# google/speedy

Hardware: AMD Instinct MI355X
Metric: Msamples/s processed (16 kHz mono, 3.5x nonlinear) (higher is better)
Workload: dtype int16 samples; f64 DFT, f32 features, int32 AMDF/OLA

## Files before the change

### speedy_amd/csrc/spx_analysis.hip

```cpp
#include <stdlib.h>

#include "spx_internal.h"
#include "spx_walk_common.h"

#ifndef SPX_TF
#define SPX_TF 16
#endif

#ifdef SPX_STAMPS
__device__ unsigned long long g_spx_astamps[16];
#define ASTAMP_DECL unsigned long long as_last = __builtin_readcyclecounter(), as_acc[10] = {0,0,0,0,0,0,0,0,0,0};
#define ASTAMP(i) do { const unsigned long long t_ = __builtin_readcyclecounter(); as_acc[i] += t_ - as_last; as_last = t_; } while (0)
#define ASTAMP_FLUSH if (threadIdx.x == 0 && blockIdx.x == 7) for (int i_ = 0; i_ < 10; i_++) g_spx_astamps[i_] += as_acc[i_];
extern "C" void spx_debug_astamps(unsigned long long* out, int reset) {
  (void)hipMemcpyFromSymbol(out, HIP_SYMBOL(g_spx_astamps), sizeof(unsigned long long) * 16);
  if (reset) { unsigned long long z[16] = {0}; (void)hipMemcpyToSymbol(HIP_SYMBOL(g_spx_astamps), z, sizeof(z)); }
}
#else
#define ASTAMP_DECL
#define ASTAMP(i)
#define ASTAMP_FLUSH
#endif

#ifndef SPX_TF_SMALL
#define SPX_TF_SMALL 8
#endif
#define SPX_TF_TINY 4
int spx_analysis_tile_frames() { return SPX_TF; }
int spx_analysis_small_tile_frames() { return SPX_TF_SMALL; }
int spx_analysis_tiny_tile_frames() { return SPX_TF_TINY; }

#define SPX_CB 24
static __host__ __device__ constexpr int spx_mag_stride(int W) { return (W + 4) & ~3; }
static __host__ __device__ constexpr int spx_cb(int tf) { return tf <= 8 ? 2 * SPX_CB : SPX_CB; }
#ifdef SPX_LOG_V1
#define SPX_LOG_LDS_BYTES 0
#else
#define SPX_LOG_LDS_BYTES 2048
#endif
static __host__ __device__ inline size_t terms_bytes(int W, int tf, bool ct) {
  const size_t b = ct ? (size_t)2 * tf * (spx_cb(tf) + 1) * sizeof(double)
                      : (size_t)tf * (W + 1) * sizeof(double);
  return (b + 15) & ~(size_t)15;
}
static __host__ __device__ inline size_t work_bytes(int W, int tf, bool ct = false, int dft_waves = 4) {
  if (dft_waves < 1 || dft_waves > 4) dft_waves = 4;
  const size_t a = ct ? (size_t)4 * 2 * W * sizeof(double)
                      : (size_t)dft_waves * 2 * 2 * W * sizeof(double);
  const size_t b = terms_bytes(W, tf, ct) + SPX_LOG_LDS_BYTES;
  return (a > b ? a : b);
}
static inline int plan_ct_window(const SpxPlanDev& P) {
  auto is = [](const int* r, int n, std::initializer_list<int> want) {
    if (n != (int)want.size()) return false;
    int k = 0;
    for (int w : want) if (r[k++] != w) return false;
    return true;
  };
  if (!P.rader && P.W == 240 && is(P.radix, P.nstages, {4, 4, 3, 5})) return 240;
  if (!P.rader && P.W == 330 && is(P.radix, P.nstages, {2, 3, 5, 11})) return 330;
  if (P.tile_frames == SPX_TF_SMALL && P.dft_waves == 4) {
    if (!P.rader && P.W == 720 && is(P.radix, P.nstages, {4, 4, 3, 3, 5})) return 720;
    if (P.rader && P.W == 661 && is(P.radixM, P.nstagesM, {4, 3, 5, 11})) return 661;
  }
  if (!P.rader && P.dft_waves == 4) {
    if (P.W == 120 && is(P.radix, P.nstages, {4, 2, 3, 5}) && (P.tile_frames == SPX_TF || P.tile_frames == SPX_TF_SMALL)) return 120;
    if (P.W == 180 && is(P.radix, P.nstages, {4, 3, 3, 5}) && P.tile_frames == SPX_TF) return 180;
    if (P.W == 360 && is(P.radix, P.nstages, {4, 2, 3, 3, 5}) && P.tile_frames == SPX_TF) return 360;
    if (P.W == 480 && is(P.radix, P.nstages, {4, 4, 2, 3, 5}) && P.tile_frames == SPX_TF) return 480;
  }
  return 0;
}
int spx_analysis_prefers_small_tile(const SpxPlanDev& P) {
  SpxPlanDev Q = P;
  Q.tile_frames = SPX_TF_SMALL;
  Q.dft_waves = 4;
  const int w = plan_ct_window(Q);
  return w == 720 || w == 661;
}
static __host__ __device__ inline size_t stage_samples(const SpxPlanDev& P, int tf) {
  return (size_t)(tf + 1) * P.B + (P.W - P.B) + 8;
}
static size_t analysis_lds_bytes(const SpxPlanDev& P, bool ct) {
  const int tf = P.tile_frames > 0 ? P.tile_frames : SPX_TF;
  size_t mags = (size_t)(tf + 1) * spx_mag_stride(P.W) * sizeof(float);
  size_t small = (size_t)3 * (tf + 1) * sizeof(float);
  size_t stage = (stage_samples(P, tf) * sizeof(short) + 15) & ~(size_t)15;
  return work_bytes(P.W, tf, ct, P.dft_waves) + ((mags + 15) & ~(size_t)15) + ((small + 15) & ~(size_t)15) + stage;
}
size_t spx_analysis_lds_bytes(const SpxPlanDev& P) { return analysis_lds_bytes(P, plan_ct_window(P) != 0); }
int spx_analysis_ct_window(const SpxPlanDev& P) { return plan_ct_window(P); }

__device__ __forceinline__ void wave_sync() {
  __builtin_amdgcn_fence(__ATOMIC_RELEASE, "wavefront");
  __builtin_amdgcn_wave_barrier();
  __builtin_amdgcn_fence(__ATOMIC_ACQUIRE, "wavefront");
}

#include "spx_log.h"

__device__ __forceinline__ float spx_untangle_mag(double ar, double ai, double b_r, double b_i, double2 w) {
  const double dr = ar - b_r, di = ai - b_i;
#ifdef SPX_DFT_V1
  const double er = 0.5 * (ar + b_r), ei = 0.5 * (ai + b_i);
  const double o_r = 0.5 * di, o_i = -0.5 * dr;
  const double xr = er + (w.x * o_r - w.y * o_i);
  const double xi = ei + (w.x * o_i + w.y * o_r);
  return spx_sqrt64_to_f32(xr * xr + xi * xi);
#else
  const double xr2 = __builtin_fma(w.x, di, __builtin_fma(w.y, dr, ar + b_r));
  const double xi2 = __builtin_fma(w.y, di, __builtin_fma(-w.x, dr, ai + b_i));
  return spx_sqrt64_to_f32(0.25 * __builtin_fma(xr2, xr2, xi2 * xi2));
#endif
}

#define C5_1 0.30901699437494742
#define C5_2 (-0.80901699437494742)
#define S5_1 0.95105651629515357
#define S5_2 0.58778525229247313
#define S3_1 0.86602540378443865

struct cplx {
  double r, i;
};

#ifdef SPX_DFT_V1
#define SPX_FMA_OR(a, b, c, unfused) (unfused)
#else
#define SPX_FMA_OR(a, b, c, unfused) __builtin_fma((a), (b), (c))
#endif
__host__ __device__ __forceinline__ cplx spx_cmul(cplx b, double wx, double wy) {
  return {SPX_FMA_OR(b.r, wx, -(b.i * wy), b.r * wx - b.i * wy), SPX_FMA_OR(b.r, wy, b.i * wx, b.r * wy + b.i * wx)};
}
__host__ __device__ __forceinline__ double spx_bf3h(double a0, double t1) { return SPX_FMA_OR(-0.5, t1, a0, a0 - 0.5 * t1); }
__host__ __device__ __forceinline__ double spx_bf5m(double a0, double c1, double t1, double c2, double t2) {
  return SPX_FMA_OR(c2, t2, __builtin_fma(c1, t1, a0), (a0 + c1 * t1) + c2 * t2);
}
__host__ __device__ __forceinline__ double spx_bf5n(double s1, double t3, double s2, double t4) { return SPX_FMA_OR(s1, t3, s2 * t4, s1 * t3 + s2 * t4); }
__host__ __device__ __forceinline__ double spx_bf5d(double s2, double t3, double s1, double t4) { return SPX_FMA_OR(s2, t3, -(s1 * t4), s2 * t3 - s1 * t4); }
__host__ __device__ __forceinline__ double spx_acc(double p, double w, double u) { return SPX_FMA_OR(w, u, p, p + w * u); }

__host__ __device__ __forceinline__ cplx ld(const double* buf, int idx) {
  const double2 v = *reinterpret_cast<const double2*>(buf + 2 * idx);
  return {v.x, v.y};
}
__host__ __device__ __forceinline__ void st_tw(double* buf, int idx, cplx b, const double* tw, int t) {
  const double2 w = *reinterpret_cast<const double2*>(tw + 2 * t);
  const cplx v = spx_cmul(b, w.x, w.y);
  *reinterpret_cast<double2*>(buf + 2 * idx) = make_double2(v.r, v.i);
}

__host__ __device__ void dft_stage(const int W, const double* tw, int r, int s, int cur, const double* x, double* y,
                                   int lane, const int nl) {
  const int m = cur / r;
  const int span = W / r;
  const unsigned inv_s = ((1u << 20) + (unsigned)s - 1u) / (unsigned)s;
  if (r == 4) {
    for (int b = lane; b < span; b += nl) {
      const int p = (int)(((unsigned)b * inv_s) >> 20), q = b - p * s;
      cplx a0 = ld(x, b), a1 = ld(x, b + span), a2 = ld(x, b + 2 * span), a3 = ld(x, b + 3 * span);
      cplx t0 = {a0.r + a2.r, a0.i + a2.i}, t1 = {a0.r - a2.r, a0.i - a2.i};
      cplx t2 = {a1.r + a3.r, a1.i + a3.i}, t3 = {a1.r - a3.r, a1.i - a3.i};
      cplx b0 = {t0.r + t2.r, t0.i + t2.i}, b2 = {t0.r - t2.r, t0.i - t2.i};
      cplx b1 = {t1.r + t3.i, t1.i - t3.r}, b3 = {t1.r - t3.i, t1.i + t3.r};
      const int o = q + s * 4 * p;
      const int tp = s * p;
      st_tw(y, o, b0, tw, 0);
      st_tw(y, o + s, b1, tw, tp);
      st_tw(y, o + 2 * s, b2, tw, 2 * tp);
      st_tw(y, o + 3 * s, b3, tw, 3 * tp);
    }
  } else if (r == 2) {
    for (int b = lane; b < span; b += nl) {
      const int p = (int)(((unsigned)b * inv_s) >> 20), q = b - p * s;
      cplx a0 = ld(x, b), a1 = ld(x, b + span);
      cplx b0 = {a0.r + a1.r, a0.i + a1.i}, b1 = {a0.r - a1.r, a0.i - a1.i};
      const int o = q + s * 2 * p;
      st_tw(y, o, b0, tw, 0);
      st_tw(y, o + s, b1, tw, s * p);
    }
  } else if (r == 3) {
    for (int b = lane; b < span; b += nl) {
      const int p = (int)(((unsigned)b * inv_s) >> 20), q = b - p * s;
      cplx a0 = ld(x, b), a1 = ld(x, b + span), a2 = ld(x, b + 2 * span);
      cplx t1 = {a1.r + a2.r, a1.i + a2.i};
      cplx t2 = {spx_bf3h(a0.r, t1.r), spx_bf3h(a0.i, t1.i)};
      cplx t3 = {S3_1 * (a1.r - a2.r), S3_1 * (a1.i - a2.i)};
      cplx b0 = {a0.r + t1.r, a0.i + t1.i};
      cplx b1 = {t2.r + t3.i, t2.i - t3.r}, b2 = {t2.r - t3.i, t2.i + t3.r};
      const int o = q + s * 3 * p;
      const int tp = s * p;
      st_tw(y, o, b0, tw, 0);
      st_tw(y, o + s, b1, tw, tp);
      st_tw(y, o + 2 * s, b2, tw, 2 * tp);
    }
  } else if (r == 5) {
    for (int b = lane; b < span; b += nl) {
      const int p = (int)(((unsigned)b * inv_s) >> 20), q = b - p * s;
      cplx a0 = ld(x, b), a1 = ld(x, b + span), a2 = ld(x, b + 2 * span), a3 = ld(x, b + 3 * span),
           a4 = ld(x, b + 4 * span);
      cplx t1 = {a1.r + a4.r, a1.i + a4.i}, t2 = {a2.r + a3.r, a2.i + a3.i};
      cplx t3 = {a1.r - a4.r, a1.i - a4.i}, t4 = {a2.r - a3.r, a2.i - a3.i};
      cplx b0 = {(a0.r + t1.r) + t2.r, (a0.i + t1.i) + t2.i};
      cplx m1 = {spx_bf5m(a0.r, C5_1, t1.r, C5_2, t2.r), spx_bf5m(a0.i, C5_1, t1.i, C5_2, t2.i)};
      cplx m2 = {spx_bf5m(a0.r, C5_2, t1.r, C5_1, t2.r), spx_bf5m(a0.i, C5_2, t1.i, C5_1, t2.i)};
      cplx n1 = {spx_bf5n(S5_1, t3.r, S5_2, t4.r), spx_bf5n(S5_1, t3.i, S5_2, t4.i)};
      cplx n2 = {spx_bf5d(S5_2, t3.r, S5_1, t4.r), spx_bf5d(S5_2, t3.i, S5_1, t4.i)};
      cplx b1 = {m1.r + n1.i, m1.i - n1.r}, b4 = {m1.r - n1.i, m1.i + n1.r};
      cplx b2 = {m2.r + n2.i, m2.i - n2.r}, b3 = {m2.r - n2.i, m2.i + n2.r};
      const int o = q + s * 5 * p;
      const int tp = s * p;
      st_tw(y, o, b0, tw, 0);
      st_tw(y, o + s, b1, tw, tp);
      st_tw(y, o + 2 * s, b2, tw, 2 * tp);
      st_tw(y, o + 3 * s, b3, tw, 3 * tp);
      st_tw(y, o + 4 * s, b4, tw, 4 * tp);
    }
  } else {
    const int step = W / r;
    const int h = (r - 1) >> 1;
    for (int item = lane; item < span * h; item += nl) {
      const int b = item / h, j = item - b * h + 1;
      const int p = (int)(((unsigned)b * inv_s) >> 20), q = b - p * s;
      const cplx a0 = ld(x, b);
      cplx P = a0, Q = {0.0, 0.0}, B0 = a0;
      int t = 0;
      for (int i = 1; i <= h; i++) {
        t += j;
        t -= (t >= r) ? r : 0;
        const cplx ai = ld(x, b + i * span), ar = ld(x, b + (r - i) * span);
        const cplx u = {ai.r + ar.r, ai.i + ar.i}, v = {ai.r - ar.r, ai.i - ar.i};
        const double2 w = *reinterpret_cast<const double2*>(tw + 2 * (t * step));
        B0.r = B0.r + u.r; B0.i = B0.i + u.i;
        P.r = spx_acc(P.r, w.x, u.r); P.i = spx_acc(P.i, w.x, u.i);
        if (i == 1) { Q.r = w.y * v.r; Q.i = w.y * v.i; }
        else { Q.r = spx_acc(Q.r, w.y, v.r); Q.i = spx_acc(Q.i, w.y, v.i); }
      }
      const cplx bj = {P.r - Q.i, P.i + Q.r}, brj = {P.r + Q.i, P.i - Q.r};
      const int o = q + s * r * p;
      st_tw(y, o + s * j, bj, tw, s * p * j);
      st_tw(y, o + s * (r - j), brj, tw, s * p * (r - j));
      if (j == 1) st_tw(y, o, B0, tw, 0);
    }
  }
  (void)m;
}

void spx_host_dft(int n, const int* radix, int nstages, const double* tw, const double* in, double* out) {
  double* a = new double[4 * (size_t)n];
  double* x = a;
  double* y = a + 2 * (size_t)n;
  for (int i = 0; i < 2 * n; i++) x[i] = in[i];
  int s = 1, cur = n;
  for (int st = 0; st < nstages; st++) {
    dft_stage(n, tw, radix[st], s, cur, x, y, 0, 1);
    double* t = x; x = y; y = t;
    s *= radix[st];
    cur /= radix[st];
  }
  for (int i = 0; i < 2 * n; i++) out[i] = x[i];
  delete[] a;
}

__device__ __forceinline__ int mono_sample(const int16_t* __restrict__ in, int64_t a, int C) {
  if (C == 1) return in[a];
  int sum = 0;
  const int16_t* p = in + a * C;
  for (int c = 0; c < C; c++) sum += p[c];
  return sum / C;
}

__device__ __forceinline__ cplx cmul_tw(cplx b, double2 w) { return spx_cmul(b, w.x, w.y); }
__device__ __forceinline__ void st(double* buf, int idx, cplx v) {
  *reinterpret_cast<double2*>(buf + 2 * idx) = make_double2(v.r, v.i);
}

template <int R>
// ... 72 lines not shown
    constexpr int SPAN = NPTS / R;
    const int b = (lane + 64 * u < SPAN) ? lane + 64 * u : 0;
    return ld(buf, b + i * SPAN);
  }
};

template <int W, int ST, int S>
__device__ __forceinline__ void ct_stages_from(double* buf, const double2* __restrict__ twp, const int lane) {
  if constexpr (ST < ct_plan<W>::n) {
    constexpr int R = ct_plan<W>::r[ST];
    ct_stage<W, R, S>(buf, twp, lane, ct_from_buf<W, R>{buf, lane});
    ct_stages_from<W, ST + 1, S * R>(buf, twp, lane);
  }
}

template <int NPTS, int R>
__device__ __forceinline__ void ct_stage_prime_last(double* buf, const int lane, const double (&wc)[R - 1], const double (&ws)[R - 1]) {
  constexpr int SPAN = NPTS / R, H = (R - 1) / 2;
  static_assert(SPAN <= 64, "one pass");
  if (lane < SPAN) {
    cplx a[R];
#pragma unroll
    for (int i = 0; i < R; i++) a[i] = ld(buf, lane + SPAN * i);
    cplx uu[H], vv[H];
    cplx B0 = a[0];
#pragma unroll
    for (int i = 1; i <= H; i++) {
      uu[i - 1] = {a[i].r + a[R - i].r, a[i].i + a[R - i].i};
      vv[i - 1] = {a[i].r - a[R - i].r, a[i].i - a[R - i].i};
      B0.r = B0.r + uu[i - 1].r; B0.i = B0.i + uu[i - 1].i;
    }
    st(buf, lane, B0);
#pragma unroll
    for (int jj = 1; jj <= H; jj++) {
      cplx Pj = a[0], Qj = {0.0, 0.0};
#pragma unroll
      for (int i = 1; i <= H; i++) {
        const double wx = wc[(i * jj) % R - 1], wy = ws[(i * jj) % R - 1];
        Pj.r = spx_acc(Pj.r, wx, uu[i - 1].r); Pj.i = spx_acc(Pj.i, wx, uu[i - 1].i);
        if (i == 1) { Qj.r = wy * vv[0].r; Qj.i = wy * vv[0].i; }
        else { Qj.r = spx_acc(Qj.r, wy, vv[i - 1].r); Qj.i = spx_acc(Qj.i, wy, vv[i - 1].i); }
      }
      st(buf, lane + SPAN * jj, cplx{Pj.r - Qj.i, Pj.i + Qj.r});
      st(buf, lane + SPAN * (R - jj), cplx{Pj.r + Qj.i, Pj.i - Qj.r});
    }
  }
  wave_sync();
}

template <class T>
__device__ __forceinline__ const T* per_frame(const T* p) {
  asm volatile("" : "+s"(p));
  return p;
}
__device__ __forceinline__ double uniform_f64(double v) {
  return __longlong_as_double(((long long)__builtin_amdgcn_readfirstlane((int)(__double_as_longlong(v) >> 32)) << 32) |
                              (unsigned)__builtin_amdgcn_readfirstlane((int)__double_as_longlong(v)));
}

#ifdef SPX_PREEMPH_V1
#define SPX_WIN_SCALE 1.0f
__device__ __forceinline__ float spx_preemph_win_f32(double md, double mpd, float w) {
  const float x = (float)(md / 32768.0), xp = (float)(mpd / 32768.0);
  const float y = (float)(1.0 * (double)x - 0.97 * (double)xp);
  return y * w;
}
#else
#define SPX_WIN_SCALE 0x1p-15f
__device__ __forceinline__ float spx_preemph_win_f32(double md, double mpd, float w15) {
  const float yy = (float)(md - 0.97 * mpd);
  return yy * w15;
}
#endif
__device__ __forceinline__ double spx_preemph_win(double md, double mpd, float w) { return (double)spx_preemph_win_f32(md, mpd, w); }
__device__ __forceinline__ cplx packed_point(const short* fr, int n, int j, int prev0, float w0, float w1) {
  const int i0 = 2 * n;
  const int m0 = fr[i0], m1 = fr[i0 + 1];
  const int mp0 = (i0 > 0) ? (int)fr[i0 - 1] : ((j > 0) ? (int)fr[prev0] : 0);
  const double d0 = (double)m0;
  return {spx_preemph_win(d0, (double)mp0, w0 * SPX_WIN_SCALE), spx_preemph_win((double)m1, d0, w1 * SPX_WIN_SCALE)};
}

#ifndef SPX_AN_W_330
#define SPX_AN_W_330 3
#endif
#ifndef SPX_AN_W_BIG
#define SPX_AN_W_BIG 2
#endif
template <int TF, int WCT>
__global__ void __launch_bounds__(SPX_BLOCK, (WCT == 240 || WCT == 120 || WCT == 180) ? 4 : WCT == 330 ? SPX_AN_W_330 : (WCT == 661 || WCT == 720) ? SPX_AN_W_BIG : (WCT == 480 || WCT == 360) ? 2 : 1)
spx_analysis_kernel(SpxPlanDev P, const SpxStreamDev* __restrict__ streams, int n_streams,
                    const int16_t* __restrict__ in_base, SpxFrameRec* __restrict__ rec, SpxTapsDev taps,
                    const int* __restrict__ tile_order, int* tile_flags, const float* __restrict__ frames,
                    int frame_mode) {
  extern __shared__ __attribute__((aligned(16))) unsigned char lds[];
  const int W = WCT ? WCT : P.W, B = P.B, N = 2 * W;
  const int tid = threadIdx.x, lane = tid & 63, wave = tid >> 6;

  const int tile = tile_order ? tile_order[blockIdx.x] : (int)blockIdx.x;
  int lo = 0, hi = n_streams - 1;
  while (lo < hi) {
    int mid = (lo + hi + 1) >> 1;
    if (streams[mid].first_tile <= tile) lo = mid; else hi = mid - 1;
  }
  const SpxStreamDev S = streams[lo];
  const int T = S.n_frames;
  const int j0 = S.frame_begin + (tile - S.first_tile) * TF;
  const int j1 = min(j0 + TF, T);
  const int C = S.channels;
  const int16_t* __restrict__ in = in_base + S.in_off;

  double* work = reinterpret_cast<double*>(lds);
  const size_t wb = work_bytes(W, TF, WCT != 0, (WCT != 0) ? 4 : P.dft_waves);
  float* mags = reinterpret_cast<float*>(lds + wb);
  const size_t mags_b = (((size_t)(TF + 1) * spx_mag_stride(W) * sizeof(float)) + 15) & ~(size_t)15;
  float* fE = reinterpret_cast<float*>(lds + wb + mags_b);
  float* fThr = fE + (TF + 1);
  float* fInv = fThr + (TF + 1);
  const int MS = spx_mag_stride(W);

  const size_t small_b = (((size_t)3 * (TF + 1) * sizeof(float)) + 15) & ~(size_t)15;
  const double* ltw = P.tw;
  const double* ltw2 = P.tw2;
  short* smono = reinterpret_cast<short*>(lds + wb + mags_b + small_b);

  double* bufA = work + (size_t)wave * (WCT != 0 ? 2 : 4) * W;
  double* bufB = (WCT != 0) ? bufA : bufA + 2 * W;

  const int jfirst = (j0 > 0) ? j0 - 1 : 0;
  const int64_t sbase = (int64_t)jfirst * B;
  const int nstage = (j1 - jfirst) * B + (W - B);
  if (frames != nullptr) {
  } else if (C == 1) {
    const int16_t* __restrict__ src = in + sbase;
    for (int k0 = tid; k0 < nstage; k0 += 8 * SPX_BLOCK) {
      short v[8];
#pragma unroll
      for (int u = 0; u < 8; u++) { const int k = k0 + u * SPX_BLOCK; v[u] = (k < nstage) ? src[k] : (short)0; }
#pragma unroll
      for (int u = 0; u < 8; u++) { const int k = k0 + u * SPX_BLOCK; if (k < nstage) smono[k] = v[u]; }
    }
  } else {
    for (int k = tid; k < nstage; k += SPX_BLOCK) smono[k] = (short)mono_sample(in, sbase + k, C);
  }
  __syncthreads();

  ASTAMP_DECL
  if constexpr (WCT == 240) {
    const double2* twp = reinterpret_cast<const double2*>(P.tw);
    const double2* tw2p = reinterpret_cast<const double2*>(P.tw2);
    const int b = lane;
    const bool on60 = b < 60, on48 = b < 48;
    const int bb = on60 ? b : 0;
    double2 w1[3], w2[3], w3[2][2], wu[4];
    float wn[4];
#pragma unroll
    for (int j = 1; j < 4; j++) { w1[j - 1] = twp[bb * j]; w2[j - 1] = twp[4 * (bb >> 2) * j]; }
#pragma unroll
    for (int u = 0; u < 2; u++) {
      const int b3 = lane + 64 * u, p3 = (b3 < 80) ? (b3 >> 4) : 0;
      w3[u][0] = twp[16 * p3];
      w3[u][1] = twp[32 * p3];
    }
#pragma unroll
    for (int u = 0; u < 4; u++) { const int k = lane + 64 * u; wu[u] = tw2p[k < 240 ? k : 0]; }
    wn[0] = P.window[2 * bb]; wn[1] = P.window[2 * bb + 1]; wn[2] = P.window[2 * bb + 120]; wn[3] = P.window[2 * bb + 121];
#pragma unroll
    for (int k = 0; k < 4; k++) wn[k] *= SPX_WIN_SCALE;
    for (int s = wave; s <= TF; s += 4) {
      const int j = j0 - 1 + s;
      float* mrow = mags + (size_t)s * MS;
      if (j < 0 || j >= j1) {
        for (int k = lane; k < 240; k += SPX_WAVE) mrow[k] = 0.0f;
        continue;
      }
      const short* fr = smono + (size_t)(j - jfirst) * B;
      if (on60) {
        const int i0 = 2 * b, i1 = 2 * b + 120;
        const int m0 = fr[i0], m1 = fr[i0 + 1], m2 = fr[i1], m3 = fr[i1 + 1];
        const int mp0 = (i0 > 0) ? (int)fr[i0 - 1] : ((j > 0) ? (int)fr[(240 - B) - 1] : 0);
        const int mp2 = fr[i1 - 1];
        const double d0 = (double)m0, d2 = (double)m2;
        const cplx a0 = {spx_preemph_win(d0, (double)mp0, wn[0]), spx_preemph_win((double)m1, d0, wn[1])},
                   a1 = {spx_preemph_win(d2, (double)mp2, wn[2]), spx_preemph_win((double)m3, d2, wn[3])};
        const cplx b0 = {a0.r + a1.r, a0.i + a1.i}, b2 = {a0.r - a1.r, a0.i - a1.i};
        const cplx b1 = {a0.r + a1.i, a0.i - a1.r}, b3 = {a0.r - a1.i, a0.i + a1.r};
        st(bufA, 4 * b, b0);
        st(bufA, 4 * b + 1, cmul_tw(b1, w1[0]));
        st(bufA, 4 * b + 2, cmul_tw(b2, w1[1]));
        st(bufA, 4 * b + 3, cmul_tw(b3, w1[2]));
      }
      wave_sync();
      ASTAMP(0);
      if (on60) {
        const cplx a0 = ld(bufA, b), a1 = ld(bufA, b + 60), a2 = ld(bufA, b + 120), a3 = ld(bufA, b + 180);
        wave_sync();
        const cplx t0 = {a0.r + a2.r, a0.i + a2.i}, t1 = {a0.r - a2.r, a0.i - a2.i};
        const cplx t2 = {a1.r + a3.r, a1.i + a3.i}, t3 = {a1.r - a3.r, a1.i - a3.i};
        const cplx b0 = {t0.r + t2.r, t0.i + t2.i}, b2 = {t0.r - t2.r, t0.i - t2.i};
        const cplx b1 = {t1.r + t3.i, t1.i - t3.r}, b3 = {t1.r - t3.i, t1.i + t3.r};
        const int o = (b & 3) + 16 * (b >> 2);
        st(bufB, o, b0);
        st(bufB, o + 4, cmul_tw(b1, w2[0]));
        st(bufB, o + 8, cmul_tw(b2, w2[1]));
        st(bufB, o + 12, cmul_tw(b3, w2[2]));
      }
      wave_sync();
      {
        cplx q0[2], q1[2], q2[2];
#pragma unroll
        for (int u = 0; u < 2; u++) {
          const int b3i = (lane + 64 * u < 80) ? lane + 64 * u : 0;
          q0[u] = ld(bufB, b3i); q1[u] = ld(bufB, b3i + 80); q2[u] = ld(bufB, b3i + 160);
        }
        wave_sync();
#pragma unroll
        for (int u = 0; u < 2; u++) {
          const int b3i = lane + 64 * u;
          if (b3i < 80) {
            const cplx a0 = q0[u], a1 = q1[u], a2 = q2[u];
            const cplx t1 = {a1.r + a2.r, a1.i + a2.i};
            const cplx t2 = {spx_bf3h(a0.r, t1.r), spx_bf3h(a0.i, t1.i)};
            const cplx t3 = {S3_1 * (a1.r - a2.r), S3_1 * (a1.i - a2.i)};
            const cplx b0 = {a0.r + t1.r, a0.i + t1.i};
            const cplx b1 = {t2.r + t3.i, t2.i - t3.r}, b2 = {t2.r - t3.i, t2.i + t3.r};
            const int o = (b3i & 15) + 48 * (b3i >> 4);
            st(bufA, o, b0);
            st(bufA, o + 16, cmul_tw(b1, w3[u][0]));
            st(bufA, o + 32, cmul_tw(b2, w3[u][1]));
          }
        }
      }
      wave_sync();
      if (on48) {
        const cplx a0 = ld(bufA, b), a1 = ld(bufA, b + 48), a2 = ld(bufA, b + 96), a3 = ld(bufA, b + 144),
                   a4 = ld(bufA, b + 192);
        wave_sync();
        const cplx t1 = {a1.r + a4.r, a1.i + a4.i}, t2 = {a2.r + a3.r, a2.i + a3.i};
        const cplx t3 = {a1.r - a4.r, a1.i - a4.i}, t4 = {a2.r - a3.r, a2.i - a3.i};
        const cplx b0 = {(a0.r + t1.r) + t2.r, (a0.i + t1.i) + t2.i};
        const cplx m1 = {spx_bf5m(a0.r, C5_1, t1.r, C5_2, t2.r), spx_bf5m(a0.i, C5_1, t1.i, C5_2, t2.i)};
        const cplx m2 = {spx_bf5m(a0.r, C5_2, t1.r, C5_1, t2.r), spx_bf5m(a0.i, C5_2, t1.i, C5_1, t2.i)};
        const cplx n1 = {spx_bf5n(S5_1, t3.r, S5_2, t4.r), spx_bf5n(S5_1, t3.i, S5_2, t4.i)};
        const cplx n2 = {spx_bf5d(S5_2, t3.r, S5_1, t4.r), spx_bf5d(S5_2, t3.i, S5_1, t4.i)};
        const cplx b1 = {m1.r + n1.i, m1.i - n1.r}, b4 = {m1.r - n1.i, m1.i + n1.r};
        const cplx b2 = {m2.r + n2.i, m2.i - n2.r}, b3 = {m2.r - n2.i, m2.i + n2.r};
        st(bufB, b, b0);
        st(bufB, b + 48, b1);
        st(bufB, b + 96, b2);
        st(bufB, b + 144, b3);
        st(bufB, b + 192, b4);
      }
      wave_sync();
      ASTAMP(1);
      float* spec_out = taps.spectrogram ? taps.spectrogram + (size_t)(S.frame_off + j) * 480 : nullptr;
#pragma unroll
      for (int u = 0; u < 4; u++) {
        const int k = lane + 64 * u;
        if (k < 240) {
          const int k2 = (k == 0) ? 0 : 240 - k;
          const cplx a = ld(bufB, k), c = ld(bufB, k2);
          const double b_r = c.r, b_i = -c.i;
          const float mag = spx_untangle_mag(a.r, a.i, b_r, b_i, wu[u]);
          mrow[k] = mag;
          if (spec_out) {
            spec_out[k] = mag;
            if (k > 0) spec_out[480 - k] = mag;
            else spec_out[240] = (float)__builtin_fabs(a.r - a.i);
          }
        }
      }
      wave_sync();
      ASTAMP(2);
    }
  } else if constexpr (WCT == 330) {
    const double2* twp = reinterpret_cast<const double2*>(P.tw);
    const double2* tw2p = reinterpret_cast<const double2*>(P.tw2);
    double2 w1[3], w2[2][2];
    float wn[3][2];
#pragma unroll
    for (int u = 0; u < 3; u++) {
      const int b1 = (lane + 64 * u < 165) ? lane + 64 * u : 0;
      w1[u] = twp[b1];
      wn[u][0] = P.window[2 * b1] * SPX_WIN_SCALE; wn[u][1] = P.window[2 * b1 + 1] * SPX_WIN_SCALE;
    }
#pragma unroll
    for (int u = 0; u < 2; u++) {
      const int p2 = (lane + 64 * u < 110) ? ((lane + 64 * u) >> 1) : 0;
      w2[u][0] = twp[2 * p2];
      w2[u][1] = twp[4 * p2];
    }
    double wc[10], ws[10];
#pragma unroll
    for (int k = 1; k <= 10; k++) {
      const double2 w = twp[k * 30];
      wc[k - 1] = __longlong_as_double(((long long)__builtin_amdgcn_readfirstlane((int)(__double_as_longlong(w.x) >> 32)) << 32) |
                                       (unsigned)__builtin_amdgcn_readfirstlane((int)__double_as_longlong(w.x)));
      ws[k - 1] = __longlong_as_double(((long long)__builtin_amdgcn_readfirstlane((int)(__double_as_longlong(w.y) >> 32)) << 32) |
                                       (unsigned)__builtin_amdgcn_readfirstlane((int)__double_as_longlong(w.y)));
    }
    for (int s = wave; s <= TF; s += 4) {
      const int j = j0 - 1 + s;
      float* mrow = mags + (size_t)s * MS;
      if (j < 0 || j >= j1) {
        for (int k = lane; k < 330; k += SPX_WAVE) mrow[k] = 0.0f;
        continue;
      }
      const short* fr = smono + (size_t)(j - jfirst) * B;
#pragma unroll
      for (int u = 0; u < 3; u++) {
        const int b = lane + 64 * u;
        if (b < 165) {
          const int i0 = 2 * b;
          const int m0 = fr[i0], m1 = fr[i0 + 1];
          const int mp0 = (i0 > 0) ? (int)fr[i0 - 1] : ((j > 0) ? (int)fr[(330 - B) - 1] : 0);
          const double d0 = (double)m0;
          const cplx a0 = {spx_preemph_win(d0, (double)mp0, wn[u][0]), spx_preemph_win((double)m1, d0, wn[u][1])};
          st(bufA, 2 * b, a0);
          st(bufA, 2 * b + 1, cmul_tw(a0, w1[u]));
        }
      }
      wave_sync();
      ASTAMP(0);
      {
        cplx q0[2], q1[2], q2[2];
#pragma unroll
        for (int u = 0; u < 2; u++) {
          const int b = (lane + 64 * u < 110) ? lane + 64 * u : 0;
          q0[u] = ld(bufA, b); q1[u] = ld(bufA, b + 110); q2[u] = ld(bufA, b + 220);
        }
        wave_sync();
#pragma unroll
        for (int u = 0; u < 2; u++) {
          const int b = lane + 64 * u;
          if (b < 110) {
            const cplx a0 = q0[u], a1 = q1[u], a2 = q2[u];
            const cplx t1 = {a1.r + a2.r, a1.i + a2.i};
            const cplx t2 = {spx_bf3h(a0.r, t1.r), spx_bf3h(a0.i, t1.i)};
            const cplx t3 = {S3_1 * (a1.r - a2.r), S3_1 * (a1.i - a2.i)};
            const cplx b0 = {a0.r + t1.r, a0.i + t1.i};
            const cplx b1 = {t2.r + t3.i, t2.i - t3.r}, b2 = {t2.r - t3.i, t2.i + t3.r};
            const int o = (b & 1) + 6 * (b >> 1);
            st(bufA, o, b0);
            st(bufA, o + 2, cmul_tw(b1, w2[u][0]));
            st(bufA, o + 4, cmul_tw(b2, w2[u][1]));
          }
        }
      }
      wave_sync();
      {
        cplx q[2][5];
#pragma unroll
        for (int u = 0; u < 2; u++) {
          const int b = (lane + 64 * u < 66) ? lane + 64 * u : 0;
#pragma unroll
          for (int i = 0; i < 5; i++) q[u][i] = ld(bufA, b + 66 * i);
        }
        wave_sync();
#pragma unroll
        for (int u = 0; u < 2; u++) {
          const int b = lane + 64 * u;
          if (b < 66) {
            const cplx a0 = q[u][0], a1 = q[u][1], a2 = q[u][2], a3 = q[u][3], a4 = q[u][4];
            const cplx t1 = {a1.r + a4.r, a1.i + a4.i}, t2 = {a2.r + a3.r, a2.i + a3.i};
            const cplx t3 = {a1.r - a4.r, a1.i - a4.i}, t4 = {a2.r - a3.r, a2.i - a3.i};
            const cplx b0 = {(a0.r + t1.r) + t2.r, (a0.i + t1.i) + t2.i};
            const cplx m1 = {spx_bf5m(a0.r, C5_1, t1.r, C5_2, t2.r), spx_bf5m(a0.i, C5_1, t1.i, C5_2, t2.i)};
            const cplx m2 = {spx_bf5m(a0.r, C5_2, t1.r, C5_1, t2.r), spx_bf5m(a0.i, C5_2, t1.i, C5_1, t2.i)};
            const cplx n1 = {spx_bf5n(S5_1, t3.r, S5_2, t4.r), spx_bf5n(S5_1, t3.i, S5_2, t4.i)};
            const cplx n2 = {spx_bf5d(S5_2, t3.r, S5_1, t4.r), spx_bf5d(S5_2, t3.i, S5_1, t4.i)};
            const cplx b1 = {m1.r + n1.i, m1.i - n1.r}, b4 = {m1.r - n1.i, m1.i + n1.r};
            const cplx b2 = {m2.r + n2.i, m2.i - n2.r}, b3 = {m2.r - n2.i, m2.i + n2.r};
            const int p = (int)(((unsigned)b * 10923u) >> 16);
            const int o = (b - 6 * p) + 30 * p, tp = 6 * p;
            st(bufA, o, b0);
            st(bufA, o + 6, cmul_tw(b1, twp[tp]));
            st(bufA, o + 12, cmul_tw(b2, twp[2 * tp]));
            st(bufA, o + 18, cmul_tw(b3, twp[3 * tp]));
            st(bufA, o + 24, cmul_tw(b4, twp[4 * tp]));
          }
        }
      }
      wave_sync();
      if (lane < 30) {
        cplx a[11];
#pragma unroll
        for (int i = 0; i < 11; i++) a[i] = ld(bufA, lane + 30 * i);
        cplx u5[5], v5[5];
        cplx B0 = a[0];
#pragma unroll
        for (int i = 1; i <= 5; i++) {
          u5[i - 1] = {a[i].r + a[11 - i].r, a[i].i + a[11 - i].i};
          v5[i - 1] = {a[i].r - a[11 - i].r, a[i].i - a[11 - i].i};
          B0.r = B0.r + u5[i - 1].r; B0.i = B0.i + u5[i - 1].i;
        }
        st(bufA, lane, B0);
#pragma unroll
        for (int jj = 1; jj <= 5; jj++) {
          cplx Pj = a[0], Qj = {0.0, 0.0};
#pragma unroll
          for (int i = 1; i <= 5; i++) {
            const double wx = wc[(i * jj) % 11 - 1], wy = ws[(i * jj) % 11 - 1];
#ifdef SPX_R11_V1
            Pj.r = Pj.r + wx * u5[i - 1].r; Pj.i = Pj.i + wx * u5[i - 1].i;
            if (i == 1) { Qj.r = wy * v5[0].r; Qj.i = wy * v5[0].i; }
            else { Qj.r = Qj.r + wy * v5[i - 1].r; Qj.i = Qj.i + wy * v5[i - 1].i; }
#else
            Pj.r = spx_acc(Pj.r, wx, u5[i - 1].r); Pj.i = spx_acc(Pj.i, wx, u5[i - 1].i);
            if (i == 1) { Qj.r = wy * v5[0].r; Qj.i = wy * v5[0].i; }
            else { Qj.r = spx_acc(Qj.r, wy, v5[i - 1].r); Qj.i = spx_acc(Qj.i, wy, v5[i - 1].i); }
#endif
          }
          st(bufA, lane + 30 * jj, cplx{Pj.r - Qj.i, Pj.i + Qj.r});
          st(bufA, lane + 30 * (11 - jj), cplx{Pj.r + Qj.i, Pj.i - Qj.r});
        }
      }
      wave_sync();
      ASTAMP(1);
      float* spec_out = taps.spectrogram ? taps.spectrogram + (size_t)(S.frame_off + j) * 660 : nullptr;
#pragma unroll
      for (int u = 0; u < 6; u++) {
// ... 174 lines not shown
    for (int i = lane; i < 2 * W; i += SPX_WAVE) {
      double v = 0.0;
      if (i < W) {
        float x, xp;
        if (frames != nullptr) {
          const float* ff = frames + (size_t)j * W;
          x = ff[i];
          if (i > 0) xp = ff[i - 1];
          else xp = (j > 0) ? ff[-1] : 0.0f;
        } else {
          const int m = fr[i];
          int mp;
          if (i > 0) mp = fr[i - 1];
          else mp = (j > 0) ? (int)fr[(W - B) - 1] : 0;
          x = (float)(m / 32768.0);
          xp = (float)(mp / 32768.0);
        }
        const float y = (frame_mode == 2) ? x : (float)(1.0 * (double)x - 0.97 * (double)xp);
        v = (double)(y * P.window[i]);
      }
      bufA[i] = v;
    }
    wave_sync();
    ASTAMP(0);
    double* x = bufA;
    double* y = bufB;
    if (P.rader) {
      const int M = W - 1;
      const cplx x0 = ld(x, 0);
      for (int p = lane; p < M; p += SPX_WAVE) {
        const cplx v = ld(x, P.perm[p]);
        *reinterpret_cast<double2*>(y + 2 * p) = make_double2(v.r, v.i);
      }
      wave_sync();
      { double* t = x; x = y; y = t; }
      for (int pass = 0; pass < 2; pass++) {
        int sprod = 1, cur = M;
        for (int stg = 0; stg < P.nstagesM; stg++) {
          const int r = P.radixM[stg];
          dft_stage(M, P.twM, r, sprod, cur, x, y, lane, SPX_WAVE);
          wave_sync();
          double* t = x; x = y; y = t;
          sprod *= r;
          cur /= r;
        }
        if (pass == 0) {
          if (lane == 0) *reinterpret_cast<double2*>(x + 2 * M) = *reinterpret_cast<const double2*>(x);
          wave_sync();
          for (int k = lane; k < M; k += SPX_WAVE) {
            const cplx a = ld(x, k);
            const double2 b = *reinterpret_cast<const double2*>(P.bfft + 2 * k);
            const cplx cc = spx_cmul(a, b.x, b.y);
            *reinterpret_cast<double2*>(x + 2 * k) = make_double2(cc.r, -cc.i);
          }
          wave_sync();
        }
      }
      const double inv = 1.0 / (double)M;
      const double* abuf = (P.nstagesM & 1) ? y : x;
      const cplx A0 = ld(abuf, M);
      wave_sync();
      for (int q = lane; q < M; q += SPX_WAVE) {
        const cplx c = ld(x, q);
        const double cr = c.r * inv, ci = -c.i * inv;
        *reinterpret_cast<double2*>(y + 2 * P.iperm[q]) = make_double2(x0.r + cr, x0.i + ci);
      }
      if (lane == 0) *reinterpret_cast<double2*>(y) = make_double2(x0.r + A0.r, x0.i + A0.i);
      wave_sync();
      { double* t = x; x = y; y = t; }
    } else {
      int sprod = 1, cur = W;
      for (int stg = 0; stg < P.nstages; stg++) {
        const int r = P.radix[stg];
        dft_stage(W, ltw, r, sprod, cur, x, y, lane, SPX_WAVE);
        wave_sync();
        double* t = x; x = y; y = t;
        sprod *= r;
        cur /= r;
      }
    }
    ASTAMP(1);
    float* spec_out = taps.spectrogram ? taps.spectrogram + (size_t)(S.frame_off + j) * N : nullptr;
    for (int k = lane; k < W; k += SPX_WAVE) {
      const int k2 = (k == 0) ? 0 : W - k;
      cplx a = ld(x, k), bb = ld(x, k2);
      const double b_r = bb.r, b_i = -bb.i;
      const float mag = spx_untangle_mag(a.r, a.i, b_r, b_i, *reinterpret_cast<const double2*>(ltw2 + 2 * k));
      mrow[k] = mag;
      if (spec_out) {
        spec_out[k] = mag;
        if (k > 0) spec_out[N - k] = mag;
        else spec_out[W] = (float)__builtin_fabs(a.r - a.i);
      }
    }
    wave_sync();
    ASTAMP(2);
  }
  ASTAMP(3);
  __syncthreads();
  ASTAMP(4);

  if (wave > 0) {
#ifdef SPX_ROWMAX_V1
    for (int s = wave - 1; s <= TF; s += 3) {
      const float* mrow = mags + (size_t)s * MS;
      float mx = 0.0f;
      for (int i = 1 + lane; i < W; i += SPX_WAVE) mx = fmaxf(mx, mrow[i]);
#pragma unroll
      for (int d = 32; d >= 1; d >>= 1) mx = fmaxf(mx, __shfl_xor(mx, d));
      if (lane == 0) fThr[s] = (float)((double)mx / 100.0);
    }
#else
    unsigned keep = 0u;
    int nrows = 0;
    for (int s = wave - 1; s <= TF; s += 3, nrows++) {
      const unsigned* mrow = reinterpret_cast<const unsigned*>(mags + (size_t)s * MS);
      unsigned m = 0u;
      for (int q = lane; 4 * q < W; q += SPX_WAVE) {
        const uint4 v = *reinterpret_cast<const uint4*>(mrow + 4 * q);
        const unsigned a = (q == 0) ? 0u : v.x;
        const unsigned b = (4 * q + 1 < W) ? v.y : 0u, c = (4 * q + 2 < W) ? v.z : 0u, d = (4 * q + 3 < W) ? v.w : 0u;
        const unsigned ab = a > b ? a : b, cd = c > d ? c : d;
        const unsigned abcd = ab > cd ? ab : cd;
        m = m > abcd ? m : abcd;
      }
      const float mx = wave_max_f(__builtin_bit_cast(float, m));
      if (lane == nrows) keep = __builtin_bit_cast(unsigned, mx);
    }
    if (lane < nrows) fThr[wave - 1 + 3 * lane] = (float)((double)__builtin_bit_cast(float, keep) / 100.0);
#endif
#ifndef SPX_LOG_V1
    if (tid < SPX_WAVE + 128)
      reinterpret_cast<uint4*>(reinterpret_cast<unsigned char*>(work) + terms_bytes(W, TF, WCT != 0))[tid - SPX_WAVE] =
          reinterpret_cast<const uint4*>(spx_log_table_dev)[tid - SPX_WAVE];
#endif
  } else if (tid <= TF) {
    const float4* r4 = reinterpret_cast<const float4*>(mags + (size_t)tid * MS);
    float e = 0.0f;
    __builtin_amdgcn_s_setprio(3);
    auto acc8 = [&](const float4& p, const float4& q) {
      const float4 pp = {p.x * p.x, p.y * p.y, p.z * p.z, p.w * p.w}, qq = {q.x * q.x, q.y * q.y, q.z * q.z, q.w * q.w};
      e += pp.x; e += pp.y; e += pp.z; e += pp.w;
      e += qq.x; e += qq.y; e += qq.z; e += qq.w;
    };
    {
      const float4 h = r4[0];
      if (1 < W) e += h.y * h.y;
      if (2 < W) e += h.z * h.z;
      if (3 < W) e += h.w * h.w;
    }
    int i = 4;
    float4 c0 = r4[1], c1 = r4[2], c2 = r4[3], c3 = r4[4];
#pragma unroll 1
    for (; i + 16 <= W; i += 16) {
      const float4 n0 = r4[(i >> 2) + 4], n1 = r4[(i >> 2) + 5], n2 = r4[(i >> 2) + 6], n3 = r4[(i >> 2) + 7];
      __builtin_amdgcn_sched_barrier(0);
      acc8(c0, c1);
      acc8(c2, c3);
      c0 = n0; c1 = n1; c2 = n2; c3 = n3;
    }
    {
      const float t[16] = {c0.x, c0.y, c0.z, c0.w, c1.x, c1.y, c1.z, c1.w, c2.x, c2.y, c2.z, c2.w, c3.x, c3.y, c3.z, c3.w};
#pragma unroll
      for (int u = 0; u < 16; u++)
        if (i + u < W) e += t[u] * t[u];
    }
    __builtin_amdgcn_s_setprio(0);
    const float eps = 2.2204e-16f;
    fE[tid] = e;
    fInv[tid] = (float)(1.0 / (__builtin_sqrt((double)e) + (double)eps));
  }
  __syncthreads();
  ASTAMP(5);

  const int nfr = j1 - j0;
#ifndef SPX_LOG_V1
  const SpxLogEntry* ltab = reinterpret_cast<const SpxLogEntry*>(reinterpret_cast<const unsigned char*>(work) + terms_bytes(W, TF, WCT != 0));
  auto log_of_ratio = [&](float ratio) -> double {
    double v = spx_log_v2_f32(ratio, ltab);
    if (__builtin_expect(!spx_log_v2_domain(ratio), 0)) v = spx_log_v1((double)ratio);
    return v;
  };
#else
  auto log_of_ratio = [&](float ratio) -> double { return spx_log_v1((double)ratio); };
#endif
  auto log_term = [&](int f, int i) -> double {
    const int sl = f + 1;
    const float cur = mags[(size_t)sl * MS + i], last = mags[(size_t)(sl - 1) * MS + i];
    const float thr = fThr[sl];
    double term = 0.0;
    if (cur > thr && last > thr) {
      const float eps = 2.2204e-16f;
      const float nc = cur * fInv[sl], nl = last * fInv[sl - 1];
      const float ratio = spx_fdiv32(nc + eps, nl + eps);
      term = __builtin_fabs(log_of_ratio(ratio));
    }
    return term;
  };
  auto write_rec = [&](int f, float lsd) {
    const float lowthr = (float)(0.04 * (double)1.41421f);
    const float e = fE[f + 1];
    SpxFrameRec r;
    r.energy = e;
    r.lsd = (e <= lowthr) ? 0.0f : lsd;
    rec[S.frame_off + j0 + f] = r;
  };
  if (taps.normalized) {
    for (int idx = tid; idx < nfr * W; idx += SPX_BLOCK) {
      const int f = idx / W, i = idx - f * W;
      const int j = j0 + f;
      const int row = j + (S.unit_time0 ? 0 : 1);
      if (row < T + (S.unit_time0 ? 1 : 0))
        taps.normalized[(size_t)(S.frame_off + row) * W + i] = mags[(size_t)(f + 1) * MS + i] * fInv[f + 1];
    }
    if (S.unit_time0) {
    } else if (j0 == 0) {
      for (int i = tid; i < W; i += SPX_BLOCK) taps.normalized[(size_t)S.frame_off * W + i] = 0.0f;
    } else if (j0 == S.frame_begin) {
      for (int i = tid; i < W; i += SPX_BLOCK)
        taps.normalized[(size_t)(S.frame_off + j0) * W + i] = mags[i] * fInv[0];
    }
  }
  if constexpr (WCT != 0) {
    constexpr int CB = spx_cb(TF);
    constexpr int CBS = CB + 1;
    static_assert(TF * CB == 2 * (SPX_BLOCK - SPX_WAVE), "two terms per lane of waves 1..3 and block");
    double* tblk = work;
    constexpr int NBLK = (WCT - 1 + CB - 1) / CB;
    float lsd = 0.0f;
    int fi[2], ci[2];
    bool ok[2];
#ifndef SPX_TERMS_V1
    const float* rowc[2];
    const float* rowl[2];
    float thrv[2], invc[2], invl[2];
#endif
#pragma unroll
    for (int t = 0; t < 2; t++) {
      const int it = tid - SPX_WAVE + t * (SPX_BLOCK - SPX_WAVE);
      fi[t] = wave > 0 ? it / CB : 0;
      ci[t] = wave > 0 ? it - fi[t] * CB : 0;
      ok[t] = wave > 0 && fi[t] < nfr;
#ifndef SPX_TERMS_V1
      const int fl = ok[t] ? fi[t] : 0;
      rowc[t] = mags + (size_t)(fl + 1) * MS;
      rowl[t] = mags + (size_t)fl * MS;
      thrv[t] = fThr[fl + 1];
      invc[t] = fInv[fl + 1];
      invl[t] = fInv[fl];
#endif
    }
    for (int k = 0; k <= NBLK; k++) {
      if (wave > 0) {
        if (k < NBLK) {
          double* tb = tblk + (size_t)(k & 1) * TF * CBS;
          bool gate[2];
          float xr[2];
#pragma unroll
          for (int t = 0; t < 2; t++) {
            const int i = 1 + k * CB + ci[t];
            const bool in = ok[t] && i < WCT;
#ifdef SPX_TERMS_V1
            const int fl = in ? fi[t] : 0, il = in ? i : 1;
            const float cur = mags[(size_t)(fl + 1) * MS + il], last = mags[(size_t)fl * MS + il];
            const float thr = fThr[fl + 1];
            const float fic = fInv[fl + 1], fil = fInv[fl];
#else
            const int il = (i < WCT) ? i : 1;
            const float cur = rowc[t][il], last = rowl[t][il];
            const float thr = thrv[t], fic = invc[t], fil = invl[t];
#endif
            gate[t] = in && cur > thr && last > thr;
            const float eps = 2.2204e-16f;
            const float nc = cur * fic, nl = last * fil;
            const float ratio = spx_fdiv32(nc + eps, nl + eps);
            xr[t] = gate[t] ? ratio : 2.0f;
          }
#ifdef SPX_LOG_V1
          const spx_log_parts p0 = spx_log_main((double)xr[0]), p1 = spx_log_main((double)xr[1]);
          const double t0 = gate[0] ? __builtin_fabs(spx_log_finish(p0, (double)xr[0])) : 0.0;
          const double t1 = gate[1] ? __builtin_fabs(spx_log_finish(p1, (double)xr[1])) : 0.0;
#else
          const double l0 = log_of_ratio(xr[0]), l1 = log_of_ratio(xr[1]);
          const double t0 = gate[0] ? __builtin_fabs(l0) : 0.0;
          const double t1 = gate[1] ? __builtin_fabs(l1) : 0.0;
#endif
          if (ok[0]) tb[fi[0] * CBS + ci[0]] = t0;
          if (ok[1]) tb[fi[1] * CBS + ci[1]] = t1;
        }
      } else if (k > 0 && tid < nfr) {
        const double* tb = tblk + (size_t)((k - 1) & 1) * TF * CBS + tid * CBS;
        const int i0 = 1 + (k - 1) * CB;
        __builtin_amdgcn_s_setprio(3);
        (void)i0;
        static_assert(CB % 8 == 0, "batches of eight");
        double tv[8];
#pragma unroll
        for (int u = 0; u < 8; u++) tv[u] = tb[u];
#pragma unroll
        for (int c = 0; c < CB; c += 8) {
          double nx[8];
          if (c + 8 < CB) {
#pragma unroll
            for (int u = 0; u < 8; u++) nx[u] = tb[c + 8 + u];
          }
#pragma unroll
          for (int u = 0; u < 8; u++) lsd = (float)((double)lsd + tv[u]);
          if (c + 8 < CB) {
#pragma unroll
            for (int u = 0; u < 8; u++) tv[u] = nx[u];
          }
        }
        __builtin_amdgcn_s_setprio(0);
      }
      ASTAMP(6);
      __syncthreads();
      ASTAMP(7);
    }
    if (tid < nfr) write_rec(tid, lsd);
  } else {
  double* terms = work;
  for (int idx = tid; idx < nfr * (W - 1); idx += SPX_BLOCK) {
    const int f = idx / (W - 1);
    const int i = 1 + (idx - f * (W - 1));
    terms[(size_t)f * (W + 1) + i] = log_term(f, i);
  }
  __syncthreads();
  ASTAMP(6);

  if (tid < nfr) {
    const double* trow = terms + (size_t)tid * (W + 1);
    float lsd = 0.0f;
    int i = 1;
    for (; i + 8 <= W; i += 8) {
      double tv[8];
#pragma unroll
      for (int u = 0; u < 8; u++) tv[u] = trow[i + u];
#pragma unroll
      for (int u = 0; u < 8; u++) lsd = (float)((double)lsd + tv[u]);
    }
    for (; i < W; i++) lsd = (float)((double)lsd + trow[i]);
    write_rec(tid, lsd);
  }
  }
  if (tile_flags) {
    asm volatile("s_waitcnt vmcnt(0)" ::: "memory");
    __syncthreads();
    if (tid == 0) {
      __builtin_amdgcn_fence(__ATOMIC_RELEASE, "agent");
      asm volatile("s_waitcnt vmcnt(0)" ::: "memory");
      __hip_atomic_store(&tile_flags[tile], 1, __ATOMIC_RELAXED, __HIP_MEMORY_SCOPE_AGENT);
    }
  }
  ASTAMP(7);
  ASTAMP_FLUSH
}

__global__ void spx_arith_check_kernel(unsigned seed, unsigned per_thread, unsigned long long* bad) {
  unsigned long long st = (unsigned long long)seed * 0x9E3779B97F4A7C15ull + (blockIdx.x * blockDim.x + threadIdx.x) * 0xD1B54A32D192ED03ull + 1;
  auto next = [&]() { st ^= st >> 12; st ^= st << 25; st ^= st >> 27; return st * 0x2545F4914F6CDD1Dull; };
  unsigned long long miss = 0;
  for (unsigned i = 0; i < per_thread; i++) {
    const unsigned long long a = next(), b = next(), c = next();
    const float fn = __uint_as_float((unsigned)((127 - 53 + (a % 57)) << 23) | (unsigned)((a >> 8) & 0x7fffff));
    const float fd = __uint_as_float((unsigned)((127 - 53 + (b % 57)) << 23) | (unsigned)((b >> 8) & 0x7fffff));
    if (__float_as_uint(spx_fdiv32(fn, fd)) != __float_as_uint(fn / fd)) miss++;
    const long long fb = ((long long)(1023 - 21 + (c % 20)) << 52) | (long long)((c >> 8) & 0xfffffffffffffll) | ((c >> 63) ? (1ll << 63) : 0);
    const double f = __longlong_as_double(fb);
    if (__double_as_longlong(spx_fdiv64(f, 2.0 + f)) != __double_as_longlong(f / (2.0 + f))) miss++;
    const long long xb = ((long long)(1023 - 800 + (a >> 33) % 1811) << 52) | (long long)((b >> 10) & 0xfffffffffffffll);
    const double x = ((c & 1023) == 0) ? 0.0 : __longlong_as_double(xb);
    if (__float_as_uint(spx_sqrt64_to_f32(x)) != __float_as_uint((float)__builtin_sqrt(x))) miss++;
  }
  if (miss) atomicAdd(bad, miss);
}
extern "C" long long spx_debug_arith_check(unsigned seed, unsigned threads, unsigned per_thread) {
  unsigned long long* d = nullptr;
  unsigned long long h = 0;
  if (hipMalloc(&d, sizeof(h)) != hipSuccess) return -1;
  if (hipMemcpy(d, &h, sizeof(h), hipMemcpyHostToDevice) != hipSuccess) { (void)hipFree(d); return -1; }
  const unsigned blocks = (threads + 255) / 256;
  hipLaunchKernelGGL(spx_arith_check_kernel, dim3(blocks), dim3(256), 0, nullptr, seed, per_thread, d);
  const bool ok = hipDeviceSynchronize() == hipSuccess && hipMemcpy(&h, d, sizeof(h), hipMemcpyDeviceToHost) == hipSuccess;
  (void)hipFree(d);
  return ok ? (long long)h : -1;
}

__global__ void __launch_bounds__(256) spx_log_check_kernel(unsigned first_block, unsigned long long* __restrict__ sums) {
#ifndef SPX_LOG_V1
  __shared__ SpxLogEntry tab[128];
  __shared__ unsigned long long acc;
  if (threadIdx.x < 128) reinterpret_cast<uint4*>(tab)[threadIdx.x] = reinterpret_cast<const uint4*>(spx_log_table_dev)[threadIdx.x];
  if (threadIdx.x == 0) acc = 0;
  __syncthreads();
  const unsigned b = first_block + blockIdx.x;
  unsigned long long sum = 0;
  for (unsigned i = threadIdx.x; i < (1u << 20); i += 256) {
    const float x = __uint_as_float((b << 20) | i);
    sum += (unsigned long long)__double_as_longlong(spx_log_v2_f32(x, tab));
  }
  atomicAdd(&acc, sum);
  __syncthreads();
  if (threadIdx.x == 0) sums[b] = acc;
#endif
}
extern "C" int spx_debug_log_check(unsigned first_block, unsigned end_block, unsigned long long* sums) {
#ifdef SPX_LOG_V1
  (void)first_block; (void)end_block; (void)sums;
  return -3;
#else
  if (first_block < 8) first_block = 8;
  if (end_block > 2040) end_block = 2040;
  if (!sums || first_block >= end_block) return -1;
  unsigned long long* d = nullptr;
  if (hipMalloc(&d, 2040 * sizeof(unsigned long long)) != hipSuccess) return -1;
  bool ok = hipMemset(d, 0, 2040 * sizeof(unsigned long long)) == hipSuccess;
  if (ok) hipLaunchKernelGGL(spx_log_check_kernel, dim3(end_block - first_block), dim3(256), 0, nullptr, first_block, d);
  ok = ok && hipDeviceSynchronize() == hipSuccess && hipMemcpy(sums, d, 2040 * sizeof(unsigned long long), hipMemcpyDeviceToHost) == hipSuccess;
  (void)hipFree(d);
  return ok ? 0 : -1;
#endif
}

void spx_launch_analysis(const SpxPlanDev& P, const SpxStreamDev* streams, int n_streams, int n_tiles,
                         const int16_t* in, SpxFrameRec* rec, SpxTapsDev taps, const int* tile_order, int* tile_flags,
                         hipStream_t st) {
  if (n_tiles <= 0) return;
  const size_t lds = spx_analysis_lds_bytes(P);
  const int ctw = plan_ct_window(P);
#define SPX_LAUNCH_ANALYSIS(TFV, WV)                                                                                   \
// ... 52 lines not shown
```

Baseline: 45270.

## Pair conjugate untangle bins, unroll energy loop, share rows across term frame pairs

```diff
diff --git a/speedy_amd/csrc/spx_analysis.hip b/speedy_amd/csrc/spx_analysis.hip
--- a/speedy_amd/csrc/spx_analysis.hip
+++ b/speedy_amd/csrc/spx_analysis.hip
@@ -123,6 +123,16 @@
 struct cplx {
   double r, i;
 };
+
+__device__ __forceinline__ void spx_untangle_mag_pair(cplx a, cplx c, double2 wk, double2 wp, float& mk, float& mp) {
+  const double dr = a.r - c.r, di = a.i + c.i, sr = a.r + c.r, si = a.i - c.i;
+  const double xr2 = __builtin_fma(wk.x, di, __builtin_fma(wk.y, dr, sr));
+  const double xi2 = __builtin_fma(wk.y, di, __builtin_fma(-wk.x, dr, si));
+  const double yr2 = __builtin_fma(wp.x, di, __builtin_fma(wp.y, -dr, sr));
+  const double yi2 = __builtin_fma(wp.y, di, __builtin_fma(-wp.x, -dr, -si));
+  mk = spx_sqrt64_to_f32(0.25 * __builtin_fma(xr2, xr2, xi2 * xi2));
+  mp = spx_sqrt64_to_f32(0.25 * __builtin_fma(yr2, yr2, yi2 * yi2));
+}
 
 #ifdef SPX_DFT_V1
 #define SPX_FMA_OR(a, b, c, unfused) (unfused)
@@ -501,7 +511,7 @@
     const int b = lane;
     const bool on60 = b < 60, on48 = b < 48;
     const int bb = on60 ? b : 0;
-    double2 w1[3], w2[3], w3[2][2], wu[4];
+    double2 w1[3], w2[3], w3[2][2], wu[2][2];
     float wn[4];
 #pragma unroll
     for (int j = 1; j < 4; j++) { w1[j - 1] = twp[bb * j]; w2[j - 1] = twp[4 * (bb >> 2) * j]; }
@@ -512,7 +522,11 @@
       w3[u][1] = twp[32 * p3];
     }
 #pragma unroll
-    for (int u = 0; u < 4; u++) { const int k = lane + 64 * u; wu[u] = tw2p[k < 240 ? k : 0]; }
+    for (int u = 0; u < 2; u++) {
+      const int k = (lane + 64 * u <= 120) ? lane + 64 * u : 0;
+      wu[u][0] = tw2p[k];
+      wu[u][1] = tw2p[k ? 240 - k : 0];
+    }
     wn[0] = P.window[2 * bb]; wn[1] = P.window[2 * bb + 1]; wn[2] = P.window[2 * bb + 120]; wn[3] = P.window[2 * bb + 121];
 #pragma unroll
     for (int k = 0; k < 4; k++) wn[k] *= SPX_WIN_SCALE;
@@ -604,18 +618,21 @@
       ASTAMP(1);
       float* spec_out = taps.spectrogram ? taps.spectrogram + (size_t)(S.frame_off + j) * 480 : nullptr;
 #pragma unroll
-      for (int u = 0; u < 4; u++) {
+      for (int u = 0; u < 2; u++) {
         const int k = lane + 64 * u;
-        if (k < 240) {
+        if (k <= 120) {
           const int k2 = (k == 0) ? 0 : 240 - k;
           const cplx a = ld(bufB, k), c = ld(bufB, k2);
-          const double b_r = c.r, b_i = -c.i;
-          const float mag = spx_untangle_mag(a.r, a.i, b_r, b_i, wu[u]);
+          float mag, mag2;
+          spx_untangle_mag_pair(a, c, wu[u][0], wu[u][1], mag, mag2);
+          const bool two = k > 0 && k < 120;
           mrow[k] = mag;
+          if (two) mrow[k2] = mag2;
           if (spec_out) {
             spec_out[k] = mag;
             if (k > 0) spec_out[480 - k] = mag;
             else spec_out[240] = (float)__builtin_fabs(a.r - a.i);
+            if (two) { spec_out[k2] = mag2; spec_out[480 - k2] = mag2; }
           }
         }
       }
@@ -1096,12 +1113,23 @@
     int i = 4;
     float4 c0 = r4[1], c1 = r4[2], c2 = r4[3], c3 = r4[4];
 #pragma unroll 1
-    for (; i + 16 <= W; i += 16) {
+    for (; i + 32 <= W; i += 32) {
+      const float4 n0 = r4[(i >> 2) + 4], n1 = r4[(i >> 2) + 5], n2 = r4[(i >> 2) + 6], n3 = r4[(i >> 2) + 7];
+      __builtin_amdgcn_sched_barrier(0);
+      acc8(c0, c1);
+      acc8(c2, c3);
+      c0 = r4[(i >> 2) + 8]; c1 = r4[(i >> 2) + 9]; c2 = r4[(i >> 2) + 10]; c3 = r4[(i >> 2) + 11];
+      __builtin_amdgcn_sched_barrier(0);
+      acc8(n0, n1);
+      acc8(n2, n3);
+    }
+    if (i + 16 <= W) {
       const float4 n0 = r4[(i >> 2) + 4], n1 = r4[(i >> 2) + 5], n2 = r4[(i >> 2) + 6], n3 = r4[(i >> 2) + 7];
       __builtin_amdgcn_sched_barrier(0);
       acc8(c0, c1);
       acc8(c2, c3);
       c0 = n0; c1 = n1; c2 = n2; c3 = n3;
+      i += 16;
     }
     {
       const float t[16] = {c0.x, c0.y, c0.z, c0.w, c1.x, c1.y, c1.z, c1.w, c2.x, c2.y, c2.z, c2.w, c3.x, c3.y, c3.z, c3.w};
@@ -1175,23 +1203,23 @@
     int fi[2], ci[2];
     bool ok[2];
 #ifndef SPX_TERMS_V1
-    const float* rowc[2];
-    const float* rowl[2];
-    float thrv[2], invc[2], invl[2];
-#endif
-#pragma unroll
-    for (int t = 0; t < 2; t++) {
-      const int it = tid - SPX_WAVE + t * (SPX_BLOCK - SPX_WAVE);
-      fi[t] = wave > 0 ? it / CB : 0;
-      ci[t] = wave > 0 ? it - fi[t] * CB : 0;
-      ok[t] = wave > 0 && fi[t] < nfr;
+    const float* rows[3];
+    float thrv[2], invs[3];
+#endif
+    {
+      const int it = wave > 0 ? tid - SPX_WAVE : 0;
+      const int g = it / CB;
+#pragma unroll
+      for (int t = 0; t < 2; t++) {
+        fi[t] = 2 * g + t;
+        ci[t] = it - g * CB;
+        ok[t] = wave > 0 && fi[t] < nfr;
+      }
 #ifndef SPX_TERMS_V1
-      const int fl = ok[t] ? fi[t] : 0;
-      rowc[t] = mags + (size_t)(fl + 1) * MS;
-      rowl[t] = mags + (size_t)fl * MS;
-      thrv[t] = fThr[fl + 1];
-      invc[t] = fInv[fl + 1];
-      invl[t] = fInv[fl];
+#pragma unroll
+      for (int r = 0; r < 3; r++) { rows[r] = mags + (size_t)(2 * g + r) * MS; invs[r] = fInv[2 * g + r]; }
+      thrv[0] = fThr[2 * g + 1];
+      thrv[1] = fThr[2 * g + 2];
 #endif
     }
     for (int k = 0; k <= NBLK; k++) {
@@ -1200,26 +1228,36 @@
           double* tb = tblk + (size_t)(k & 1) * TF * CBS;
           bool gate[2];
           float xr[2];
+          const float eps = 2.2204e-16f;
+#ifdef SPX_TERMS_V1
 #pragma unroll
           for (int t = 0; t < 2; t++) {
             const int i = 1 + k * CB + ci[t];
             const bool in = ok[t] && i < WCT;
-#ifdef SPX_TERMS_V1
             const int fl = in ? fi[t] : 0, il = in ? i : 1;
             const float cur = mags[(size_t)(fl + 1) * MS + il], last = mags[(size_t)fl * MS + il];
             const float thr = fThr[fl + 1];
             const float fic = fInv[fl + 1], fil = fInv[fl];
-#else
-            const int il = (i < WCT) ? i : 1;
-            const float cur = rowc[t][il], last = rowl[t][il];
-            const float thr = thrv[t], fic = invc[t], fil = invl[t];
-#endif
             gate[t] = in && cur > thr && last > thr;
-            const float eps = 2.2204e-16f;
             const float nc = cur * fic, nl = last * fil;
             const float ratio = spx_fdiv32(nc + eps, nl + eps);
             xr[t] = gate[t] ? ratio : 2.0f;
           }
+#else
+          {
+            const int i = 1 + k * CB + ci[0];
+            const int il = (i < WCT) ? i : 1;
+            float m[3], n[3];
+#pragma unroll
+            for (int r = 0; r < 3; r++) { m[r] = rows[r][il]; n[r] = m[r] * invs[r] + eps; }
+#pragma unroll
+            for (int t = 0; t < 2; t++) {
+              gate[t] = ok[t] && i < WCT && m[t + 1] > thrv[t] && m[t] > thrv[t];
+              const float ratio = spx_fdiv32(n[t + 1], n[t]);
+              xr[t] = gate[t] ? ratio : 2.0f;
+            }
+          }
+#endif
 #ifdef SPX_LOG_V1
           const spx_log_parts p0 = spx_log_main((double)xr[0]), p1 = spx_log_main((double)xr[1]);
           const double t0 = gate[0] ? __builtin_fabs(spx_log_finish(p0, (double)xr[0])) : 0.0;
```

Result: no change. 45430 (median of 6 runs) (+0.3%).
